# saltoricristiano/lidog

Hardware: AMD Instinct MI355X
Metric: LiDAR scans/sec, MinkUNet34+BEV training step @120k pts (higher is better)
Workload: dtype f32

## Files before the change

include/lidog_amd.h:

```cpp
#ifndef LIDOG_AMD_H
#define LIDOG_AMD_H

#include <stdint.h>

#ifdef __cplusplus
extern "C" {
#endif

const char *lidog_last_error(void);
int lidog_abi_version(void);


int64_t lidog_hash_capacity(int64_t n);

int lidog_coords_insert(const int32_t *coords, int64_t n, uint64_t *keys, int32_t *vals, int64_t cap,
                        int32_t *first_row, int64_t *n_unique_dev, int32_t *err_flag, void *stream);
int lidog_coords_insert_info(const int32_t *coords, int64_t n, uint64_t *keys, int32_t *vals, int64_t cap,
                             int32_t *first_row, int64_t *info, int32_t *err_flag, void *stream);

int lidog_coords_compact(const int32_t *first_row, int64_t n, const uint64_t *keys, int32_t *vals, int64_t cap,
                         const int32_t *coords, int32_t *unique_rows, int32_t *inverse, int32_t *scan_ws,
                         void *stream);

int lidog_coords_stride(const int32_t *coords_in, int64_t n_in, int32_t new_stride, uint64_t *keys,
                        int32_t *vals, int64_t cap, int32_t *parent2child, int32_t *coords_out,
                        int64_t *n_out_dev, int32_t *ws, int32_t *err_flag, void *stream);

int64_t lidog_bitmap_words(int32_t nx, int32_t ny, int32_t nz, int32_t nb, int64_t max_bytes);
int lidog_bitmap_set(const int32_t *coords, int64_t n, int32_t x0, int32_t y0, int32_t z0, int32_t nx, int32_t ny,
                     int32_t nz, int32_t stride, int32_t nb, uint32_t *bits, int32_t *err_flag, void *stream);
int lidog_kernel_map_bits(const int32_t *coords_out, int64_t n_out, const uint64_t *in_keys, const int32_t *in_vals,
                          int64_t in_cap, const int32_t *offsets_host, int32_t K, const uint32_t *bits, int32_t x0,
                          int32_t y0, int32_t z0, int32_t nx, int32_t ny, int32_t nz, int32_t stride, int32_t nb,
                          int32_t *nbr, void *stream);
int lidog_kernel_map_subset(const int32_t *nbr_big, int64_t n, int32_t K_big, const int32_t *sel_host, int32_t K,
                            int32_t *nbr, void *stream);

int lidog_kernel_map(const int32_t *coords_out, int64_t n_out, const uint64_t *in_keys, const int32_t *in_vals,
                     int64_t in_cap, const int32_t *offsets_host, int32_t K, int32_t *nbr, void *stream);

int lidog_kernel_map_pairs(const int32_t *nbr, int64_t n_out, int64_t n_in, int32_t K, int64_t *k_off_dev,
                           int32_t *pair_in, int32_t *pair_out, int32_t *pos_out, int32_t *pos_in, int32_t *ws,
                           void *stream);
int lidog_kernel_map_rows(const int32_t *pos, int64_t n, int32_t K, int32_t mark_k, int32_t *row_ptr,
                          int32_t *row_list, int32_t *ws, void *stream);


int lidog_sconv_gemm(const float *A, const int32_t *gather, const float *B, const float *bias,
                     const int32_t *tile_k, const int32_t *tile_row0, const int32_t *tile_rows, int32_t n_tiles,
                     int32_t Cin, int32_t Cout, float *T, const int32_t *scatter, int64_t a_rows, void *stream);
int32_t lidog_sconv_gemm_units(int32_t multi, int32_t slots);
int lidog_sconv_gemm_addend(const float *A, const int32_t *gather, const float *B, const int32_t *tile_k,
                            const int32_t *tile_row0, const int32_t *tile_rows, int32_t n_tiles, int32_t Cin,
                            int32_t Cout, const float *addend, float *T, const int32_t *scatter, void *stream);

int lidog_sconv_reduce(const float *T, const int32_t *pos, int64_t n, int32_t K, int32_t C, const float *bias,
                       const float *addend ,
                       float *out, void *stream);

int64_t lidog_sconv_reduce_stats_ws(int64_t n, int32_t C);
int lidog_sconv_reduce_stats(const float *T, const int32_t *pos, int64_t n, int32_t K, int32_t C, const float *bias,
                             float *out, double *sums, double *partial_ws, double count, float eps, float momentum,
                             float *mean, float *invstd, float *running_mean, float *running_var, void *stream);
int lidog_sconv_reduce_rows(const float *T, const int32_t *row_ptr, const int32_t *row_list, int64_t n, int32_t C,
                            const float *bias, const float *addend, float *out, void *stream);
int lidog_sconv_reduce_rows_stats(const float *T, const int32_t *row_ptr, const int32_t *row_list, int64_t n,
                                  int32_t C, const float *bias, float *out, double *sums, double *partial_ws,
                                  double count, float eps, float momentum, float *mean, float *invstd,
                                  float *running_mean, float *running_var, void *stream);
int lidog_sconv_reduce_rows_bwdstats(const float *T, const int32_t *row_ptr, const int32_t *row_list, int64_t n,
                                     int32_t C, const float *addend, float *out, const float *pre,
                                     const float *relu_y, const uint32_t *relu_bits, const float *mean,
                                     const float *invstd, const float *relu_w, const float *relu_b, double *sums,
                                     double *partial_ws, double count, float *dw, float *db, void *stream);
int lidog_sconv_reduce_rows_bn(const float *T, const int32_t *row_ptr, const int32_t *row_list, int64_t n, int32_t C,
                               const float *bias, const float *mean, const float *invstd, const float *w,
                               const float *b, const float *residual, int32_t relu, float *out, void *stream);

int lidog_sconv_cin1(const float *x, const int32_t *nbr, const float *W, const float *bias, int64_t n, int32_t K,
                     int32_t C, float *out, void *stream);

int lidog_sconv_wgrad(const float *A, const int32_t *pair_a, const float *G, const int32_t *pair_g,
                      const int32_t *items, int32_t n_items, const int32_t *item_off, int32_t K, int32_t Cin,
                      int32_t Cout, float *partial, float *gW, void *stream);

int lidog_sconv_wgrad_slabs(int32_t Cin, int32_t Cout, int32_t n_items);
int32_t lidog_sconv_wgrad_slots(int32_t Cin, int32_t Cout, int32_t fold);

int lidog_set_sparse_core(int32_t core);
int lidog_get_sparse_core(void);

int lidog_transpose_kernel(const float *W, int32_t K, int32_t Cin, int32_t Cout, float *Wt, void *stream);
int lidog_transpose_batched(const float *src, float *dst, const int64_t *desc, int32_t n_mats, int64_t total_tiles,
                            void *stream);


int64_t lidog_bn_reduce_ws(int32_t C, int64_t hw);
int lidog_bn_stats(const float *x, int64_t n, int32_t C, int64_t hw, double *sums, double *ws, double count,
                   float eps, float momentum, float *mean, float *invstd, float *running_mean, float *running_var,
                   void *stream);
int lidog_bn_finalize(const double *sums, double count, int32_t C, float eps, float momentum, float *mean,
                      float *invstd, float *running_mean, float *running_var, void *stream);
int lidog_bn_apply(const float *x, int64_t n, int32_t C, int64_t hw, const float *mean, const float *invstd,
                   const float *w, const float *b, const float *residual, int32_t relu, float *y, void *stream);
int32_t lidog_stats_max_blocks(void);
int64_t lidog_bn_bwd_reduce_blocks(int64_t n, int32_t C);
int lidog_bn_bwd_reduce(const float *dy, const float *x, const float *relu_y, int64_t n, int32_t C, int64_t hw,
                        const float *mean, const float *invstd, double *sums, double *ws, double count, float *dw,
                        float *db, const float *relu_w, const float *relu_b, void *stream);
int lidog_bn_bwd_apply(const float *dy, const float *x, const float *relu_y, int64_t n, int32_t C, int64_t hw,
                       const float *mean, const float *invstd, const float *w, const double *sums, double count,
                       float *dx, float *dres, float *dw, float *db, const float *relu_b, void *stream);
int64_t lidog_relu_bits_words(int64_t n, int32_t C);
int lidog_bn_apply_bits(const float *x, int64_t n, int32_t C, int64_t hw, const float *mean, const float *invstd,
                        const float *w, const float *b, const float *residual, int32_t relu, float *y,
                        uint32_t *relu_bits, void *stream);
int lidog_bn_apply_sync(const float *x, int64_t n, int32_t C, const double *sums, float eps, float momentum, float *mean,
                        float *invstd, float *running_mean, float *running_var, const float *w, const float *b,
                        const float *residual, int32_t relu, float *y, uint32_t *relu_bits, void *stream);
int lidog_bn_bwd_reduce_bits(const float *dy, const float *x, const float *relu_y, const uint32_t *relu_bits, int64_t n,
                             int32_t C, int64_t hw, const float *mean, const float *invstd, double *sums, double *ws,
                             double count, float *dw, float *db, const float *relu_w, const float *relu_b,
                             void *stream);
int lidog_bn_bwd_apply_bits(const float *dy, const float *x, const float *relu_y, const uint32_t *relu_bits, int64_t n,
                            int32_t C, int64_t hw, const float *mean, const float *invstd, const float *w,
                            const double *sums, double count, float *dx, float *dres, float *dw, float *db,
                            const float *relu_b, void *stream);
int lidog_colsum(const float *x, int64_t n, int32_t C, float *out, double *ws, void *stream);
int64_t lidog_colsum_ws(int32_t C);
int lidog_bn_eval_invstd(const float *running_var, float eps, int32_t C, float *invstd, void *stream);
int lidog_cat2(const float *a, int32_t Ca, const float *b, int32_t Cb, int64_t n, float *out, void *stream);
int lidog_split2(const float *g, int32_t Ca, int32_t Cb, int64_t n, float *ga, float *gb, void *stream);
int lidog_relu_fwd(const float *x, int64_t n, float *y, void *stream);
int lidog_relu_bwd(const float *dy, const float *y, int64_t n, float *dx, void *stream);
int lidog_add(const float *a, const float *b, int64_t n, float *out, void *stream);

int lidog_bev_winner(const int32_t *coords, int64_t n, const int32_t *lut_x, const int32_t *lut_y, int32_t lut_lo,
                     int32_t lut_n, int32_t H, int32_t W, int32_t *winner ,
                     int32_t *pixel , void *stream);
int lidog_bev_pool_fwd(const float *feats, int32_t C, const int32_t *winner, const int32_t *pixel, int64_t n,
                       int32_t B, int32_t H, int32_t W, int32_t pk, int32_t ps, int32_t pp, int32_t Ho, int32_t Wo,
                       float *out ,
                       int32_t *argsrc , uint64_t *rowbits,
                       void *stream);
int lidog_bev_pool_bwd(const float *gout , const int32_t *argsrc, const int32_t *winner,
                       const int32_t *pixel, int64_t n, int32_t C, int32_t B, int32_t H, int32_t W, int32_t pk,
                       int32_t ps, int32_t pp, int32_t Ho, int32_t Wo, float *gfeats , void *stream);

int lidog_conv2d_fwd(const float *x, const float *w, const float *bias, int32_t B, int32_t Cin, int32_t H,
                     int32_t W, int32_t Cout, int32_t ksize, int32_t stride, int32_t pad, float *y, void *stream);
int lidog_conv2d_dgrad(const float *gy, const float *w, int32_t B, int32_t Cin, int32_t H, int32_t W,
                       int32_t Cout, int32_t ksize, int32_t stride, int32_t pad, float *gx, float *ws,
                       void *stream);
int lidog_conv2d_wgrad(const float *x, const float *gy, int32_t B, int32_t Cin, int32_t H, int32_t W,
                       int32_t Cout, int32_t ksize, int32_t stride, int32_t pad, float *gw, float *gbias,
                       float *ws, int64_t ws_floats, void *stream);

int64_t lidog_conv2d_support_ws(int32_t B, int32_t Cin, int32_t H, int32_t W);
int lidog_conv2d_support(const int32_t *support, int32_t B, int32_t Cin, int32_t H, int32_t W, int32_t *act,
                         void *stream);
int lidog_conv2d_fwd_sparse(const float *x, const float *w, const int32_t *act, int32_t B, int32_t Cin, int32_t H,
                            int32_t W, int32_t Cout, float *y, float *ws, void *stream);
int lidog_conv2d_dgrad_sparse(const float *gy, const float *w, const int32_t *act, int32_t B, int32_t Cin, int32_t H,
                              int32_t W, int32_t Cout, float *gx, float *ws, void *stream);
int lidog_conv2d_support_work(const int32_t *act, int32_t B, int32_t Cin, int32_t H, int32_t W, int32_t Cout,
                              double *out, void *stream);
int64_t lidog_conv2d_wgrad_sparse_ws(int32_t B, int32_t Cin, int32_t H, int32_t W, int32_t Cout);
int lidog_conv2d_wgrad_sparse(const float *x, const float *gy, const int32_t *act, int32_t B, int32_t Cin, int32_t H,
                              int32_t W, int32_t Cout, float *gw, float *ws, int64_t ws_floats, void *stream);

int64_t lidog_dice_ws(int32_t C);
int lidog_dice_fwd(const float *logits, const int64_t *target, int64_t n, int32_t C, int64_t ignore_label,
                   int32_t has_ignore, float eps, int32_t soft, int32_t powerize, int32_t use_tmask, float offset,
                   double *ws, float *loss, float *coef, void *stream);
int lidog_dice_bwd(const float *logits, const int64_t *target, int64_t n, int32_t C, int64_t ignore_label,
                   int32_t has_ignore, float eps, int32_t soft, int32_t powerize, const float *coef, const float *gout,
                   float *glogits, void *stream);
int lidog_dice_kitti_fwd(const float *logits, const int64_t *target, int64_t n, int32_t C, int64_t ignore_label,
                         int32_t has_ignore, float eps, int32_t powerize, int32_t use_tmask, float offset, double *ws,
                         float *loss, float *coef, void *stream);
int lidog_dice_kitti_bwd(const float *logits, const int64_t *target, int64_t n, int32_t C, int64_t ignore_label,
                         int32_t has_ignore, float eps, int32_t powerize, const float *coef, const float *gout,
                         float *glogits, void *stream);

int64_t lidog_ce_ws(int32_t C);
int lidog_ce_fwd(const float *logits, const int64_t *target, int64_t n, int32_t C, int64_t ignore_label,
                 int32_t has_ignore, const float *weight, int32_t focal, double alpha, double gamma, double *ws,
                 float *loss, float *coef, void *stream);
int lidog_ce_bwd(const float *logits, const int64_t *target, int64_t n, int32_t C, int64_t ignore_label,
                 int32_t has_ignore, const float *weight, const float *coef, const float *gout, float *glogits,
                 void *stream);

int lidog_voxel_floor(const float *points, int64_t n, float qx, float qy, float qz, int32_t batch, int32_t *rows,
                      void *stream);
int lidog_label_vote(const int32_t *labels, const int32_t *unique_rows, const int32_t *inverse, int64_t n, int64_t m,
                     int32_t ignore_label, int32_t *voxel_labels, void *stream);
int lidog_bev_label_raster(const int32_t *coords, const int32_t *labels, int64_t n, const int32_t *lut_x,
                           const int32_t *lut_y, const int32_t *lut_z, int32_t lut_lo, int32_t lut_n, int32_t B,
                           int32_t S, const int64_t *batch_start, int32_t *point_idx, int64_t *img_labels,
                           void *stream);

int lidog_adam_step(float *param, const float *grad, float *exp_avg, float *exp_avg_sq, int64_t n, float lr,
                    float beta1, float beta2, float eps, float weight_decay, int32_t step, float grad_scale,
                    void *stream);
int lidog_grad_accumulate(const int64_t *segs, int32_t n_segs, void *stream);
int lidog_sgd_step(float *param, const float *grad, float *momentum_buf, int64_t n, float lr, float momentum,
                   float weight_decay, int32_t nesterov, float grad_scale, void *stream);

int32_t lidog_comm_unique_id_bytes(void);
int lidog_comm_unique_id(void *id_out);
int lidog_comm_init_rank(const void *id, int32_t nranks, int32_t rank, void **comm_out);
int lidog_comm_destroy(void *comm);
int32_t lidog_comm_count(void *comm);
int lidog_allreduce_f32(float *buf, int64_t n, void *comm, void *stream);
int lidog_allreduce_f64(double *buf, int64_t n, void *comm, void *stream);

int32_t lidog_peer_handle_bytes(void);
int64_t lidog_peer_mailbox_bytes(int32_t nranks, int32_t max_doubles);
int lidog_peer_mailbox_alloc(int64_t bytes, void **ptr_out, void *handle_out);
int lidog_peer_mailbox_open(const void *handle, void **ptr_out);
int lidog_peer_comm_create(int32_t rank, int32_t nranks, int32_t max_doubles, void *local, void *const *peer_ptrs,
                           void **comm_out);
int32_t lidog_peer_max_doubles(void *comm);
int lidog_peer_set_spin_limit(void *comm, int64_t polls );
int lidog_peer_allreduce_f64(void *comm, double *buf, int64_t n, void *stream);
int32_t lidog_peer_status(void *comm);
int lidog_peer_comm_destroy(void *comm, int32_t close_peers);
int lidog_peer_rebind_stream(void *comm, void *stream);
int64_t lidog_peer_calls(void *comm);
int lidog_peer_inject_skip_flag(void *comm, int64_t seq);
int lidog_peer_mailbox_free(void *ptr);
int lidog_peer_mailbox_close(void *peer_ptr);

int64_t lidog_kernel_map_sorted_ws(int64_t n);
int lidog_kernel_map_sorted(const int32_t *nbr, int64_t n, int32_t K, const int64_t *k_off, int32_t *perm,
                            uint32_t *wave_masks, int32_t *tile_order, void *ws, int64_t ws_bytes, void *stream);
int lidog_sconv_os(const float *A, const int32_t *nbr, int64_t n, int32_t K, const int32_t *perm,
                   const uint32_t *wave_masks, const int32_t *tile_order, const float *W, int32_t reverse,
                   const float *bias, const float *addend, int32_t Cin, int32_t Cout, float *out, void *stream);
int64_t lidog_sconv_os_stats_ws(int64_t n, int32_t C);
// ... 178 lines not shown
```

lidog_amd/_lib.py:

```python
import ctypes
import os

import torch

_HERE = os.path.dirname(os.path.abspath(__file__))
SO_PATH = os.environ.get("LIDOG_SO") or os.path.join(_HERE, "_C", "liblidog_amd.so")

_i32, _i64, _p, _f, _d = ctypes.c_int32, ctypes.c_int64, ctypes.c_void_p, ctypes.c_float, ctypes.c_double

SIGNATURES = {
    "lidog_abi_version": [],
    "lidog_hash_capacity": [_i64],
    "lidog_coords_insert": [_p, _i64, _p, _p, _i64, _p, _p, _p, _p],
    "lidog_coords_insert_info": [_p, _i64, _p, _p, _i64, _p, _p, _p, _p],
    "lidog_coords_compact": [_p, _i64, _p, _p, _i64, _p, _p, _p, _p, _p],
    "lidog_coords_stride": [_p, _i64, _i32, _p, _p, _i64, _p, _p, _p, _p, _p, _p],
    "lidog_kernel_map": [_p, _i64, _p, _p, _i64, _p, _i32, _p, _p],
    "lidog_bitmap_words": [_i32, _i32, _i32, _i32, _i64],
    "lidog_bitmap_set": [_p, _i64, _i32, _i32, _i32, _i32, _i32, _i32, _i32, _i32, _p, _p, _p],
    "lidog_kernel_map_bits": [_p, _i64, _p, _p, _i64, _p, _i32, _p, _i32, _i32, _i32, _i32, _i32, _i32, _i32, _i32, _p, _p],
    "lidog_kernel_map_pairs": [_p, _i64, _i64, _i32, _p, _p, _p, _p, _p, _p, _p],
    "lidog_sconv_gemm_units": [_i32, _i32],
    "lidog_sconv_gemm": [_p, _p, _p, _p, _p, _p, _p, _i32, _i32, _i32, _p, _p, _i64, _p],
    "lidog_sconv_gemm_addend": [_p, _p, _p, _p, _p, _p, _i32, _i32, _i32, _p, _p, _p, _p],
    "lidog_sconv_reduce": [_p, _p, _i64, _i32, _i32, _p, _p, _p, _p],
    "lidog_sconv_reduce_stats_ws": [_i64, _i32],
    "lidog_sconv_reduce_stats": [_p, _p, _i64, _i32, _i32, _p, _p, _p, _p, _d, _f, _f, _p, _p, _p, _p, _p],
    "lidog_kernel_map_rows": [_p, _i64, _i32, _i32, _p, _p, _p, _p],
    "lidog_sconv_reduce_rows": [_p, _p, _p, _i64, _i32, _p, _p, _p, _p],
    "lidog_sconv_reduce_rows_bn": [_p, _p, _p, _i64, _i32, _p, _p, _p, _p, _p, _p, _i32, _p, _p],
    "lidog_sconv_reduce_rows_stats": [_p, _p, _p, _i64, _i32, _p, _p, _p, _p, _d, _f, _f, _p, _p, _p, _p, _p],
    "lidog_sconv_reduce_rows_bwdstats": [_p, _p, _p, _i64, _i32, _p, _p, _p, _p, _p, _p, _p, _p, _p, _p, _p, _d, _p, _p, _p],
    "lidog_bn_bwd_reduce_blocks": [_i64, _i32],
    "lidog_stats_max_blocks": [],
    "lidog_sconv_cin1": [_p, _p, _p, _p, _i64, _i32, _i32, _p, _p],
    "lidog_kernel_map_subset": [_p, _i64, _i32, _p, _i32, _p, _p],
    "lidog_kernel_map_sorted_ws": [_i64],
    "lidog_kernel_map_sorted": [_p, _i64, _i32, _p, _p, _p, _p, _p, _i64, _p],
    "lidog_sconv_os": [_p, _p, _i64, _i32, _p, _p, _p, _p, _i32, _p, _p, _i32, _i32, _p, _p],
    "lidog_sconv_os_stats_ws": [_i64, _i32],
    "lidog_sconv_os_bn": [_p, _p, _i64, _i32, _p, _p, _p, _p, _p, _i32, _i32, _p, _p, _p, _p, _p, _i32, _p, _p],
    "lidog_sconv_os_stats": [_p, _p, _i64, _i32, _p, _p, _p, _p, _p, _i32, _i32, _p, _p, _p, _d, _f, _f, _p, _p, _p, _p, _p],
    "lidog_pack_kernels_bf16": [_p, _p, _p, _i32, _i64, _p],
    "lidog_sconv_gemm_bf16": [_p, _p, _p, _p, _p, _p, _p, _i32, _i32, _i32, _p, _p, _p],
    "lidog_sconv_os_bn_bf16": [_p, _p, _i64, _i32, _p, _p, _p, _p, _p, _i32, _i32, _p, _p, _p, _p, _p, _i32, _p, _p],
    "lidog_sconv_wgrad_bf16": [_p, _p, _p, _p, _p, _i32, _p, _i32, _i32, _i32, _p, _p, _p],
    "lidog_sconv_wgrad_bf16_slabs": [_i32, _i32, _i32],
    "lidog_sconv_wgrad_bf16_slots": [_i32, _i32],
    "lidog_sconv_wgrad": [_p, _p, _p, _p, _p, _i32, _p, _i32, _i32, _i32, _p, _p, _p],
    "lidog_sconv_gemm_in_bn": [_p, _p, _p, _p, _p, _p, _p, _i32, _i32, _i32, _p, _p, _p, _p, _p, _p, _i32, _i64, _p],
    "lidog_sconv_os_stats_in_bn": [_p, _p, _i64, _i32, _p, _p, _p, _p, _p, _i32, _i32, _p, _p, _p, _d, _f, _f, _p, _p, _p, _p,
                                   _p, _p, _p, _p, _i32, _p],
    "lidog_sconv_wgrad_in_bn": [_p, _p, _p, _p, _p, _i32, _p, _i32, _i32, _i32, _p, _p, _p, _p, _p, _p, _i32, _p],
    "lidog_sconv_wgrad_slabs": [_i32, _i32, _i32],
    "lidog_sconv_wgrad_slots": [_i32, _i32, _i32],
    "lidog_set_sparse_core": [_i32],
    "lidog_get_sparse_core": [],
    "lidog_transpose_kernel": [_p, _i32, _i32, _i32, _p, _p],
    "lidog_transpose_batched": [_p, _p, _p, _i32, _i64, _p],
    "lidog_bn_reduce_ws": [_i32, _i64],
    "lidog_bn_stats": [_p, _i64, _i32, _i64, _p, _p, _d, _f, _f, _p, _p, _p, _p, _p],
    "lidog_bn_finalize": [_p, _d, _i32, _f, _f, _p, _p, _p, _p, _p],
    "lidog_bn_apply": [_p, _i64, _i32, _i64, _p, _p, _p, _p, _p, _i32, _p, _p],
    "lidog_bn_bwd_reduce": [_p, _p, _p, _i64, _i32, _i64, _p, _p, _p, _p, _d, _p, _p, _p, _p, _p],
    "lidog_bn_bwd_apply": [_p, _p, _p, _i64, _i32, _i64, _p, _p, _p, _p, _d, _p, _p, _p, _p, _p, _p],
    "lidog_relu_bits_words": [_i64, _i32],
    "lidog_bn_apply_bits": [_p, _i64, _i32, _i64, _p, _p, _p, _p, _p, _i32, _p, _p, _p],
    "lidog_bn_bwd_reduce_bits": [_p, _p, _p, _p, _i64, _i32, _i64, _p, _p, _p, _p, _d, _p, _p, _p, _p, _p],
    "lidog_bn_bwd_apply_bits": [_p, _p, _p, _p, _i64, _i32, _i64, _p, _p, _p, _p, _d, _p, _p, _p, _p, _p, _p],
    "lidog_colsum": [_p, _i64, _i32, _p, _p, _p],
    "lidog_colsum_ws": [_i32],
    "lidog_bn_eval_invstd": [_p, _f, _i32, _p, _p],
    "lidog_cat2": [_p, _i32, _p, _i32, _i64, _p, _p],
    "lidog_split2": [_p, _i32, _i32, _i64, _p, _p, _p],
    "lidog_relu_fwd": [_p, _i64, _p, _p],
    "lidog_relu_bwd": [_p, _p, _i64, _p, _p],
    "lidog_add": [_p, _p, _i64, _p, _p],
    "lidog_bev_winner": [_p, _i64, _p, _p, _i32, _i32, _i32, _i32, _p, _p, _p],
    "lidog_bev_pool_fwd": [_p, _i32, _p, _p, _i64, _i32, _i32, _i32, _i32, _i32, _i32, _i32, _i32, _p, _p, _p, _p],
    "lidog_bev_pool_bwd": [_p, _p, _p, _p, _i64, _i32, _i32, _i32, _i32, _i32, _i32, _i32, _i32, _i32, _p, _p],
    "lidog_conv2d_fwd": [_p, _p, _p, _i32, _i32, _i32, _i32, _i32, _i32, _i32, _i32, _p, _p],
    "lidog_conv2d_dgrad": [_p, _p, _i32, _i32, _i32, _i32, _i32, _i32, _i32, _i32, _p, _p, _p],
    "lidog_conv2d_wgrad": [_p, _p, _i32, _i32, _i32, _i32, _i32, _i32, _i32, _i32, _p, _p, _p, _i64, _p],
    "lidog_conv2d_support_ws": [_i32, _i32, _i32, _i32],
    "lidog_conv2d_support": [_p, _i32, _i32, _i32, _i32, _p, _p],
    "lidog_conv2d_fwd_sparse": [_p, _p, _p, _i32, _i32, _i32, _i32, _i32, _p, _p, _p],
    "lidog_conv2d_dgrad_sparse": [_p, _p, _p, _i32, _i32, _i32, _i32, _i32, _p, _p, _p],
    "lidog_conv2d_wgrad_sparse_ws": [_i32, _i32, _i32, _i32, _i32],
    "lidog_conv2d_wgrad_sparse": [_p, _p, _p, _i32, _i32, _i32, _i32, _i32, _p, _p, _i64, _p],
    "lidog_voxel_floor": [_p, _i64, _f, _f, _f, _i32, _p, _p],
    "lidog_label_vote": [_p, _p, _p, _i64, _i64, _i32, _p, _p],
    "lidog_bev_label_raster": [_p, _p, _i64, _p, _p, _p, _i32, _i32, _i32, _i32, _p, _p, _p, _p],
    "lidog_dice_ws": [_i32],
    "lidog_dice_fwd": [_p, _p, _i64, _i32, _i64, _i32, _f, _i32, _i32, _i32, _f, _p, _p, _p, _p],
    "lidog_dice_bwd": [_p, _p, _i64, _i32, _i64, _i32, _f, _i32, _i32, _p, _p, _p, _p],
    "lidog_dice_kitti_fwd": [_p, _p, _i64, _i32, _i64, _i32, _f, _i32, _i32, _f, _p, _p, _p, _p],
    "lidog_dice_kitti_bwd": [_p, _p, _i64, _i32, _i64, _i32, _f, _i32, _p, _p, _p, _p],
    "lidog_ce_ws": [_i32],
    "lidog_ce_fwd": [_p, _p, _i64, _i32, _i64, _i32, _p, _i32, _d, _d, _p, _p, _p, _p],
    "lidog_ce_bwd": [_p, _p, _i64, _i32, _i64, _i32, _p, _p, _p, _p, _p],
    "lidog_adam_step": [_p, _p, _p, _p, _i64, _f, _f, _f, _f, _f, _i32, _f, _p],
    "lidog_sgd_step": [_p, _p, _p, _i64, _f, _f, _f, _i32, _f, _p],
    "lidog_comm_unique_id_bytes": [],
    "lidog_comm_unique_id": [_p],
    "lidog_comm_init_rank": [_p, _i32, _i32, ctypes.POINTER(ctypes.c_void_p)],
    "lidog_comm_destroy": [_p],
    "lidog_allreduce_f32": [_p, _i64, _p, _p],
    "lidog_allreduce_f64": [_p, _i64, _p, _p],
    "lidog_comm_count": [_p],
    "lidog_peer_handle_bytes": [],
    "lidog_peer_mailbox_bytes": [_i32, _i32],
    "lidog_peer_mailbox_alloc": [_i64, ctypes.POINTER(ctypes.c_void_p), _p],
    "lidog_peer_mailbox_open": [_p, ctypes.POINTER(ctypes.c_void_p)],
    "lidog_peer_comm_create": [_i32, _i32, _i32, _p, _p, ctypes.POINTER(ctypes.c_void_p)],
    "lidog_peer_max_doubles": [_p],
    "lidog_peer_set_spin_limit": [_p, _i64],
    "lidog_peer_allreduce_f64": [_p, _p, _i64, _p],
    "lidog_peer_status": [_p],
    "lidog_peer_comm_destroy": [_p, _i32],
    "lidog_peer_rebind_stream": [_p, _p],
    "lidog_peer_calls": [_p],
    "lidog_peer_inject_skip_flag": [_p, _i64],
    "lidog_peer_mailbox_free": [_p],
    "lidog_peer_mailbox_close": [_p],
    "lidog_tiles_host": [_p, _i32, _i32, _i32, _p, _i64],
    "lidog_wgrad_items_host": [_p, _i32, _i64, _i32, _i32, _p, _p, _i64],
    "lidog_conv2d_support_work": [_p, _i32, _i32, _i32, _i32, _i32, _p, _p],
    "lidog_bn_apply_sync": [_p, _i64, _i32, _p, _f, _f, _p, _p, _p, _p, _p, _p, _p, _i32, _p, _p, _p],
    "lidog_trunk_fusions": [_i32],
    "lidog_trunk_in_bn_readers": [_p, _i32, _p, _i32, _p, _i32, _p, _i32, _p],
    "lidog_trunk_gemm_timing": [_i32],
    "lidog_trunk_gemm_timing_read": [_p],
    "lidog_trunk_work_read": [_p],
    "lidog_trunk_forward": [_p, _p, _i32, _p, _i32, _p, _i32, _p, _i32, _p, _p, _p, _i64, _p, _i64, _p, _p, _i32, _p, _p, _p],
    "lidog_trunk_backward": [_p, _p, _i32, _p, _i32, _p, _i32, _p, _i32, _p, _p, _p, _p, _p, _p, _i64, _p, _i64, _p,
                             _i64, _p, _p, _i32, _i32, _p, _p, _p],
    "lidog_in_segments_ws": [_i64],
    "lidog_in_segments": [_p, _i64, _i32, _p, _p, _p, _p, _i64, _p],
    "lidog_in_reduce_ws": [_i32, _i32],
    "lidog_in_stats": [_p, _i64, _i32, _i32, _p, _p, _f, _p, _p, _p, _p],
    "lidog_in_apply": [_p, _i64, _i32, _i32, _p, _p, _p, _p, _p, _p, _p],
    "lidog_in_bwd_reduce": [_p, _p, _i64, _i32, _i32, _p, _p, _p, _p, _p, _p, _p, _p, _p],
    "lidog_in_bwd_apply": [_p, _p, _i64, _i32, _i32, _p, _p, _p, _p, _p, _p, _p],
    "lidog_ibn_apply": [_p, _i64, _i32, _i32, _p, _p, _p, _p, _p, _p, _p, _p, _p, _p, _p, _p],
    "lidog_ibn_bwd_reduce": [_p, _p, _p, _i64, _i32, _i32, _p, _p, _p, _p, _p, _p, _p, _p, _p, _p, _p, _p, _p, _p, _p],
    "lidog_ibn_bwd_apply": [_p, _p, _p, _i64, _i32, _i32, _p, _p, _p, _p, _d, _p, _p, _p, _p, _p, _p, _p],
    "lidog_iw_ws": [],
    "lidog_iw_fwd": [_p, _p, _p, _p, _i32, _d, _p, _p, _p, _p],
    "lidog_iw_bwd": [_p, _p, _p, _p, _i32, _d, _p, _p, _p],
    "lidog_grad_accumulate": [_p, _i32, _p],
    "lidog_mix_histogram": [_p, _i64, _i32, _p, _p],
    "lidog_mix_split_ws": [_i64, _i32],
    "lidog_mix_split": [_p, _i64, _p, _i32, _i32, _p, _p, _p, _p],
    "lidog_mix_gather": [_p, _i64, _p, _p, _p, _p, _p, _i32, _i64, _f, _p, _i32, _p, _p, _p],
    "lidog_mix_gather_aug": [_p, _i64, _p, _i64, _p, _p, _p, _p, _i32, _i64, _f, _p, _i32, _p, _i32, _d, _d, _d, _p, _i32,
                             _p, _p, _p],
    "lidog_dbscan_ws": [_i64],
    "lidog_dbscan": [_p, _i64, _f, _d, _i32, _p, _p, _p, _i64, _p],
    "lidog_cluster_boxes": [_p, _p, _i64, _i32, _p, _p, _p, _p],
    "lidog_sn_scale_coords": [_p, _i64, _f, _f, _f, _f, _p, _p],
    "lidog_augment_is_f64": [_p, _i32],
    "lidog_augment_ws": [_i64],
    "lidog_augment_points": [_p, _i64, _p, _i64, _p, _p, _i32, _i32, _d, _d, _d, _i32, _p, _p, _p, _p, _p, _p, _p, _p],
    "lidog_eval_confusion": [_p, _p, _p, _i64, _i32, _i32, _i64, _p, _p, _p, _p],
    "lidog_eval_pack_ws": [_i64, _i32],
    "lidog_eval_pack": [_p, _p, _p, _i64, _i32, _i64, _p, _p, _p, _p],
    "lidog_train_confusion": [_p, _p, _p, _i32, _i32, _i64, _p, _p, _p],
    "lidog_scan_load_ws": [_i64],
    "lidog_scan_load": [_p, _i32, _p, _i32, _i32, _i64, _p, _i32, _i32, _f, _p, _p, _p, _i32, _p, _p, _p],
    "lidog_scan_keep_rows_ws": [_i64],
    "lidog_scan_keep_rows": [_p, _i32, _i64, _i32, _f, _p, _p, _p, _p],
    "lidog_point_labels_ws": [_i64],
    "lidog_point_labels": [_p, _i64, _i32, _i32, _p, _p, _p, _i64, _i64, _p, _p, _p, ctypes.c_uint32, _p, _i32, _i32, _p,
                           _i32, _i64, _p, _p, _p, _p, _p],
    "lidog_pool_rows": [_p, _p, _p, _p, _i64, _i32, _i32, _p, _p, _p],
    "lidog_pool_rows_max": [_p, _p, _p, _p, _i64, _i32, _p, _p, _p],
    "lidog_pool_rows_max_bwd": [_p, _p, _p, _p, _p, _i64, _i32, _p, _p],
    "lidog_pool_global_ws": [_i64, _i32, _i32],
    "lidog_pool_global": [_p, _i64, _i32, _i32, _p, _p, _i32, _p, _p, _p, _i64, _p],
    "lidog_pool_global_bwd": [_p, _p, _i64, _i32, _i32, _p, _p, _i32, _p, _p],
}
_RESTYPES = {"lidog_hash_capacity": _i64, "lidog_sconv_reduce_stats_ws": _i64, "lidog_bn_reduce_ws": _i64,
             "lidog_dice_ws": _i64, "lidog_ce_ws": _i64, "lidog_colsum_ws": _i64, "lidog_conv2d_support_ws": _i64, "lidog_conv2d_wgrad_sparse_ws": _i64,
             "lidog_tiles_host": _i64, "lidog_wgrad_items_host": _i64, "lidog_bitmap_words": _i64,
             "lidog_bn_bwd_reduce_blocks": _i64, "lidog_relu_bits_words": _i64,
             "lidog_peer_mailbox_bytes": _i64, "lidog_peer_calls": _i64,
             "lidog_kernel_map_sorted_ws": _i64, "lidog_sconv_os_stats_ws": _i64, "lidog_in_segments_ws": _i64,
             "lidog_in_reduce_ws": _i64, "lidog_iw_ws": _i64, "lidog_mix_split_ws": _i64,
             "lidog_dbscan_ws": _i64, "lidog_augment_ws": _i64, "lidog_eval_pack_ws": _i64,
             "lidog_scan_load_ws": _i64, "lidog_pool_global_ws": _i64, "lidog_scan_keep_rows_ws": _i64,
             "lidog_point_labels_ws": _i64}

ABI_VERSION = 8

_lib = None


def load():
    global _lib
    if _lib is None:
        if not os.path.exists(SO_PATH):
            raise RuntimeError(
                f"{SO_PATH} is missing: build it with `python -m lidog_amd.build` (hipcc, gfx950). "
                "lidog_amd has no CPU or torch fallback.")
        L = ctypes.CDLL(SO_PATH)
        L.lidog_last_error.restype = ctypes.c_char_p
        L.lidog_last_error.argtypes = []
        have = L.lidog_abi_version()
# ... 52 lines not shown
```

lidog_amd/csrc/sconv_mfma.hip:

```cpp
#include <stdlib.h>

#include "common.h"
#include "sconv_mfma.h"
#include "clock_stamp.h"

typedef float f32x16 __attribute__((ext_vector_type(16)));

#define MG_TM 128
#define MG_BK 32
#define MG_SA 33

template <int NT>
__device__ __forceinline__ void frag_load(const float *p, float (&f)[NT]) {
    if constexpr (NT == 4) {
        float4 v = *reinterpret_cast<const float4 *>(p);
        f[0] = v.x; f[1] = v.y; f[2] = v.z; f[3] = v.w;
    } else if constexpr (NT == 2) {
        float2 v = *reinterpret_cast<const float2 *>(p);
        f[0] = v.x; f[1] = v.y;
    } else {
#pragma unroll
        for (int t = 0; t < NT; ++t) f[t] = p[t];
    }
}
// ... 461 lines not shown
    constexpr int TPW = (TILES + WPG - 1) / WPG;
    __shared__ __attribute__((aligned(16))) float As[MW_R * TM];
    __shared__ __attribute__((aligned(16))) float Gs[MW_R * TN];
    const int item = items[3 * n_items + blockIdx.x];
    const int tiles_n = Cout / TN;
    const int ci0 = (blockIdx.y / tiles_n) * TM, co0 = (blockIdx.y % tiles_n) * TN;
    const int tid = threadIdx.x, lane = tid & 63, wave = tid >> 6;
    const int li = lane & 31, kh = lane >> 5;
    LIDOG_STAMP_BEGIN()
    const int grp = wave / WPG, wig = wave % WPG;
    const int64_t p0 = items[n_items + item], p1 = items[2 * n_items + item];

    int a_off[TPW], g_off[TPW];
    bool own[TPW];
#pragma unroll
    for (int t = 0; t < TPW; ++t) {
        int tt = wig * TPW + t;
        own[t] = tt < TILES;
        int mi = own[t] ? tt % MT : 0, nj = own[t] ? tt / MT : 0;
        a_off[t] = 32 * mi + li;
        g_off[t] = 32 * nj + li;
    }
    f32x16 acc[TPW];
#pragma unroll
    for (int t = 0; t < TPW; ++t)
#pragma unroll
        for (int e = 0; e < 16; ++e) acc[t][e] = 0.f;

    constexpr int AV = (MW_R * TM / 4 + NTH - 1) / NTH, GV = (MW_R * TN / 4 + NTH - 1) / NTH;
    float4 ra[AV], rg[GV];
    int ia[AV], ig[GV];
    auto load_idx = [&](int64_t p) {
#pragma unroll
        for (int j = 0; j < AV; ++j) {
            int f = tid + NTH * j;
            f = f < MW_R * TM / 4 ? f : MW_R * TM / 4 - 1;
            int64_t pr = p + f / (TM / 4);
            ia[j] = pa[pr < p1 ? pr : p1 - 1];
        }
#pragma unroll
        for (int j = 0; j < GV; ++j) {
            int f = tid + NTH * j;
            f = f < MW_R * TN / 4 ? f : MW_R * TN / 4 - 1;
            int64_t pr = p + f / (TN / 4);
            ig[j] = pg[pr < p1 ? pr : p1 - 1];
        }
    };
    auto load_rows = [&](int64_t p) {
#pragma unroll
        for (int j = 0; j < AV; ++j) {
            int f = tid + NTH * j;
            f = f < MW_R * TM / 4 ? f : MW_R * TM / 4 - 1;
            int r = f / (TM / 4), c4 = f % (TM / 4);
            (void)r;
            ra[j] = *reinterpret_cast<const float4 *>(A + (size_t)ia[j] * Cin + ci0 + c4 * 4);
        }
#pragma unroll
        for (int j = 0; j < GV; ++j) {
            int f = tid + NTH * j;
            f = f < MW_R * TN / 4 ? f : MW_R * TN / 4 - 1;
            int r = f / (TN / 4), c4 = f % (TN / 4);
            (void)r;
            rg[j] = *reinterpret_cast<const float4 *>(G + (size_t)ig[j] * Cout + co0 + c4 * 4);
        }
    };
    if (p0 < p1) {
        load_idx(p0);
        load_rows(p0);
        load_idx(p0 + MW_R);
    }
    if constexpr (FOLD) {
        for (int i = tid; i < TM; i += NTH) {
            s_par[i] = in_bn.mean[ci0 + i];
            s_par[TM + i] = in_bn.invstd[ci0 + i];
            s_par[2 * TM + i] = in_bn.w[ci0 + i];
            s_par[3 * TM + i] = in_bn.b[ci0 + i];
        }
    }
    for (int64_t p = p0; p < p1; p += MW_R) {
        __syncthreads();
#pragma unroll
        for (int j = 0; j < AV; ++j) {
            int f = tid + NTH * j;
            const bool ok = p + f / (TM / 4) < p1;
            float4 v = ra[j];
            if constexpr (FOLD) {
                const int c = ((f < MW_R * TM / 4 ? f : MW_R * TM / 4 - 1) % (TM / 4)) * 4;
                v = in_bn_apply(v, *reinterpret_cast<const float4 *>(&s_par[c]),
                                *reinterpret_cast<const float4 *>(&s_par[TM + c]),
                                *reinterpret_cast<const float4 *>(&s_par[2 * TM + c]),
                                *reinterpret_cast<const float4 *>(&s_par[3 * TM + c]), in_bn.relu);
            }
            if (f < MW_R * TM / 4) *reinterpret_cast<float4 *>(&As[f * 4]) = make_float4(ok ? v.x : 0.f, ok ? v.y : 0.f, ok ? v.z : 0.f, ok ? v.w : 0.f);
        }
#pragma unroll
        for (int j = 0; j < GV; ++j) {
            int f = tid + NTH * j;
            const bool ok = p + f / (TN / 4) < p1;
            if (f < MW_R * TN / 4) *reinterpret_cast<float4 *>(&Gs[f * 4]) = make_float4(ok ? rg[j].x : 0.f, ok ? rg[j].y : 0.f, ok ? rg[j].z : 0.f, ok ? rg[j].w : 0.f);
        }
        __syncthreads();
        if (p + MW_R < p1) {
            load_rows(p + MW_R);
            load_idx(p + 2 * MW_R);
        }
        constexpr int Q = MW_R / 2 / NGRP;
        float af[TPW], gf[TPW], an[TPW], gn[TPW];
        {
            const int kk = 2 * grp + kh;
#pragma unroll
            for (int t = 0; t < TPW; ++t) {
                af[t] = As[kk * TM + a_off[t]];
                gf[t] = Gs[kk * TN + g_off[t]];
            }
        }
#pragma unroll
        for (int q = 0; q < Q; ++q) {
            if (q + 1 < Q) {
                const int kk = 2 * ((q + 1) * NGRP + grp) + kh;
#pragma unroll
                for (int t = 0; t < TPW; ++t) {
                    an[t] = As[kk * TM + a_off[t]];
                    gn[t] = Gs[kk * TN + g_off[t]];
                }
            }
            __builtin_amdgcn_sched_barrier(0);
#pragma unroll
            for (int t = 0; t < TPW; ++t) acc[t] = __builtin_amdgcn_mfma_f32_32x32x2f32(af[t], gf[t], acc[t], 0, 0, 0);
            __builtin_amdgcn_sched_barrier(0);
            if (q + 1 < Q) {
#pragma unroll
                for (int t = 0; t < TPW; ++t) {
                    af[t] = an[t];
                    gf[t] = gn[t];
                }
            }
        }
    }
    float *dst = partial + (size_t)(item * NGRP + grp) * Cin * Cout;
#pragma unroll
    for (int t = 0; t < TPW; ++t) {
        if (!own[t]) continue;
        int tt = wig * TPW + t;
        int mi = tt % MT, nj = tt / MT;
#pragma unroll
        for (int e = 0; e < 16; ++e) {
            int ci = ci0 + 32 * mi + (e & 3) + 8 * (e >> 2) + 4 * kh;
            dst[(size_t)ci * Cout + co0 + 32 * nj + li] = acc[t][e];
        }
    }
    LIDOG_STAMP_END()
}

static int tile32(int C) { return (C % 128 == 0) ? 4 : (C % 96 == 0) ? 3 : (C % 64 == 0) ? 2 : 1; }

static void wg_shape(int tiles, int *nw, int *ngrp) {
    switch (tiles) {
        case 1: *nw = 4; *ngrp = 4; break;
        case 2: *nw = 4; *ngrp = 2; break;
        case 3: case 6: case 9: *nw = 3; *ngrp = 1; break;
        default: *nw = 4; *ngrp = 1;
    }
}

int lidog_wgrad_mfma_slabs(int Cin, int Cout, int n_items) {
    int nw, ngrp;
    wg_shape(tile32(Cin) * tile32(Cout), &nw, &ngrp);
    return n_items * ngrp;
}

template <int MT, int NT, int NW, int NGRP>
static void launch_wg(dim3 grid, hipStream_t st, const float *A, const int32_t *pa, const float *G, const int32_t *pg,
                      const int32_t *items, int n_items, int Cin, int Cout, float *partial, InBn in_bn) {
    if (in_bn.mean)
        k_sconv_wgrad_mfma<MT, NT, NW, NGRP, true><<<grid, 64 * NW, 0, st>>>(A, pa, G, pg, items, n_items, Cin, Cout,
                                                                             partial, in_bn);
    else
        k_sconv_wgrad_mfma<MT, NT, NW, NGRP, false><<<grid, 64 * NW, 0, st>>>(A, pa, G, pg, items, n_items, Cin, Cout,
                                                                              partial, in_bn);
}

template <int MT, int NT, int NW, int NGRP>
static int occ_wg(bool fold) {
    int n = 0;
    hipError_t e = fold ? hipOccupancyMaxActiveBlocksPerMultiprocessor(&n, k_sconv_wgrad_mfma<MT, NT, NW, NGRP, true>, 64 * NW, 0)
                        : hipOccupancyMaxActiveBlocksPerMultiprocessor(&n, k_sconv_wgrad_mfma<MT, NT, NW, NGRP, false>, 64 * NW, 0);
    return e == hipSuccess ? n : -1;
}

int lidog_wgrad_mfma_wg_per_cu(int Cin, int Cout, int fold) {
    int mt = tile32(Cin), nt = tile32(Cout);
#define WG(MT_, NT_, NW_, NG_) return occ_wg<MT_, NT_, NW_, NG_>(fold != 0)
    switch (mt * 10 + nt) {
        case 11: WG(1, 1, 4, 4);
        case 12: WG(1, 2, 4, 2);
        case 21: WG(2, 1, 4, 2);
        case 13: WG(1, 3, 3, 1);
        case 31: WG(3, 1, 3, 1);
        case 14: WG(1, 4, 4, 1);
        case 41: WG(4, 1, 4, 1);
        case 22: WG(2, 2, 4, 1);
        case 23: WG(2, 3, 3, 1);
        case 32: WG(3, 2, 3, 1);
        case 24: WG(2, 4, 4, 1);
        case 42: WG(4, 2, 4, 1);
        case 33: WG(3, 3, 3, 1);
        case 34: WG(3, 4, 4, 1);
        case 43: WG(4, 3, 4, 1);
        default: WG(4, 4, 4, 1);
    }
#undef WG
}

int lidog_launch_wgrad_mfma(const float *A, const int32_t *pa, const float *G, const int32_t *pg,
                            const int32_t *items, int n_items, int Cin, int Cout, float *partial, InBn in_bn,
                            hipStream_t st) {
    int mt = tile32(Cin), nt = tile32(Cout);
    dim3 grid((unsigned)n_items, (unsigned)((Cin / (32 * mt)) * (Cout / (32 * nt))));
#define WG(MT_, NT_, NW_, NG_) launch_wg<MT_, NT_, NW_, NG_>(grid, st, A, pa, G, pg, items, n_items, Cin, Cout, partial, in_bn)
    switch (mt * 10 + nt) {
        case 11: WG(1, 1, 4, 4); break;
        case 12: WG(1, 2, 4, 2); break;
        case 21: WG(2, 1, 4, 2); break;
        case 13: WG(1, 3, 3, 1); break;
        case 31: WG(3, 1, 3, 1); break;
        case 14: WG(1, 4, 4, 1); break;
        case 41: WG(4, 1, 4, 1); break;
        case 22: WG(2, 2, 4, 1); break;
        case 23: WG(2, 3, 3, 1); break;
        case 32: WG(3, 2, 3, 1); break;
        case 24: WG(2, 4, 4, 1); break;
        case 42: WG(4, 2, 4, 1); break;
        case 33: WG(3, 3, 3, 1); break;
        case 34: WG(3, 4, 4, 1); break;
        case 43: WG(4, 3, 4, 1); break;
        default: WG(4, 4, 4, 1);
    }
#undef WG
    return 0;
}
```

Before: 86.71.

## Add LDS ring-buffered wgrad MFMA kernel with async global-to-LDS DMA for 32x32

Adds a new weight-gradient kernel that stages gathered A and G rows into a multi-stage LDS ring using global_load_lds direct DMA, with pair indices prefetched ahead and row loads interleaved between MFMA issues. Out-of-range rows read from a device zero row. By default it is selected only for non-folded Cin=Cout=32 layers, and a runtime override picks 2 or 3 stages. The aim is to hide gather latency behind MFMA work, at the cost of more LDS use, hand-written waitcnt bookkeeping and possibly lower occupancy.

After: 86.73, median of 4. No clear change (+0.0%).

```diff
diff --git a/include/lidog_amd.h b/include/lidog_amd.h
--- a/include/lidog_amd.h
+++ b/include/lidog_amd.h
@@ -86,6 +86,9 @@
 
 int lidog_sconv_wgrad_slabs(int32_t Cin, int32_t Cout, int32_t n_items);
 int32_t lidog_sconv_wgrad_slots(int32_t Cin, int32_t Cout, int32_t fold);
+
+int32_t lidog_sconv_wgrad_ring(int32_t form);
+int32_t lidog_zero_row_nonzeros(void);
 
 int lidog_set_sparse_core(int32_t core);
 int lidog_get_sparse_core(void);
diff --git a/lidog_amd/_lib.py b/lidog_amd/_lib.py
--- a/lidog_amd/_lib.py
+++ b/lidog_amd/_lib.py
@@ -54,6 +54,8 @@
     "lidog_sconv_wgrad_in_bn": [_p, _p, _p, _p, _p, _i32, _p, _i32, _i32, _i32, _p, _p, _p, _p, _p, _p, _i32, _p],
     "lidog_sconv_wgrad_slabs": [_i32, _i32, _i32],
     "lidog_sconv_wgrad_slots": [_i32, _i32, _i32],
+    "lidog_sconv_wgrad_ring": [_i32],
+    "lidog_zero_row_nonzeros": [],
     "lidog_set_sparse_core": [_i32],
     "lidog_get_sparse_core": [],
     "lidog_transpose_kernel": [_p, _i32, _i32, _i32, _p, _p],
diff --git a/lidog_amd/csrc/sconv_mfma.hip b/lidog_amd/csrc/sconv_mfma.hip
--- a/lidog_amd/csrc/sconv_mfma.hip
+++ b/lidog_amd/csrc/sconv_mfma.hip
@@ -637,6 +637,224 @@
     LIDOG_STAMP_END()
 }
 
+
+__device__ __attribute__((aligned(16))) float g_zero_row[128];
+
+extern "C" int32_t lidog_zero_row_nonzeros(void) {
+    uint32_t host[128];
+    if (hipMemcpyFromSymbol(host, HIP_SYMBOL(g_zero_row), sizeof(host)) != hipSuccess) return -1;
+    int32_t n = 0;
+    for (int i = 0; i < 128; ++i) n += host[i] != 0u;
+    return n;
+}
+
+__device__ __forceinline__ unsigned ring_lds_addr(const void *p) {
+    return __builtin_amdgcn_readfirstlane((unsigned)(size_t)(__attribute__((address_space(3))) const char *)p);
+}
+__device__ __forceinline__ void ring_dma16(const void *gsrc, unsigned lds_dst) {
+    unsigned keep;
+    asm volatile("s_mov_b32 %0, m0\n\ts_mov_b32 m0, %2\n\ts_nop 0\n\tglobal_load_lds_dwordx4 %1, off\n\ts_mov_b32 m0, %0"
+                 : "=&s"(keep) : "v"(gsrc), "s"(lds_dst) : "memory");
+}
+__device__ __forceinline__ void ring_dma4(const void *gsrc, unsigned lds_dst) {
+    unsigned keep;
+    asm volatile("s_mov_b32 %0, m0\n\ts_mov_b32 m0, %2\n\ts_nop 0\n\tglobal_load_lds_dword %1, off\n\ts_mov_b32 m0, %0"
+                 : "=&s"(keep) : "v"(gsrc), "s"(lds_dst) : "memory");
+}
+#define RING_MAX_WAIT 24
+__device__ __forceinline__ void ring_wait_vm(int n) {
+#define RW(N_) case N_: asm volatile("s_waitcnt vmcnt(" #N_ ")" ::: "memory"); break;
+    switch (n) {
+        RW(1) RW(2) RW(3) RW(4) RW(5) RW(6) RW(7) RW(8) RW(9) RW(10) RW(11) RW(12)
+        RW(13) RW(14) RW(15) RW(16) RW(17) RW(18) RW(19) RW(20) RW(21) RW(22) RW(23) RW(24)
+        default: asm volatile("s_waitcnt vmcnt(0)" ::: "memory");
+    }
+#undef RW
+}
+__device__ __forceinline__ void ring_barrier() { asm volatile("s_waitcnt lgkmcnt(0)\n\ts_barrier" ::: "memory"); }
+
+template <int MT, int NT, int NW, int NGRP, bool FOLD, int R, int S>
+__global__ __launch_bounds__(64 * NW) void k_sconv_wgrad_ring(const float *__restrict__ A, const int32_t *__restrict__ pa,
+                                                              const float *__restrict__ G, const int32_t *__restrict__ pg,
+                                                              const int32_t *__restrict__ items, int n_items, int Cin,
+                                                              int Cout, float *__restrict__ partial, InBn in_bn) {
+    constexpr int TM = 32 * MT, TN = 32 * NT, NTH = 64 * NW;
+    constexpr int TILES = MT * NT;
+    constexpr int WPG = NW / NGRP, TPW = (TILES + WPG - 1) / WPG;
+    constexpr int PA = R * TM / 256, PG = R * TN / 256;
+    constexpr int AV = (PA + NW - 1) / NW, GV = (PG + NW - 1) / NW;
+    constexpr int LA = S - 1;
+    constexpr int NI = 8;
+    static_assert(R % (2 * NGRP) == 0 && R <= 32 && LA >= 1 && LA <= 3 && LA + 2 <= NI, "ring shape");
+    static_assert((LA - 1) * (AV + GV + 1) <= RING_MAX_WAIT, "ring_wait_vm range");
+    __shared__ __attribute__((aligned(1024))) float As[S * R * TM];
+    __shared__ __attribute__((aligned(1024))) float Gs[S * R * TN];
+    __shared__ __attribute__((aligned(256))) int32_t Is[NI * 64];
+    __shared__ __attribute__((aligned(16))) float s_par[FOLD ? 4 * TM : 4];
+    const int item = items[3 * n_items + blockIdx.x];
+    const int tiles_n = Cout / TN;
+    const int ci0 = (blockIdx.y / tiles_n) * TM, co0 = (blockIdx.y % tiles_n) * TN;
+    const int tid = threadIdx.x, lane = tid & 63, wave = __builtin_amdgcn_readfirstlane(tid >> 6);
+    const int li = lane & 31, kh = lane >> 5;
+    LIDOG_STAMP_BEGIN()
+    const int grp = wave / WPG, wig = wave % WPG;
+    const int64_t p0 = items[n_items + item], p1 = items[2 * n_items + item];
+    const int nc = p0 < p1 ? (int)((p1 - p0 + R - 1) / R) : 0;
+
+    int a_off[TPW], g_off[TPW];
+    bool own[TPW];
+#pragma unroll
+    for (int t = 0; t < TPW; ++t) {
+        int tt = wig * TPW + t;
+        own[t] = tt < TILES;
+        int mi = own[t] ? tt % MT : 0, nj = own[t] ? tt / MT : 0;
+        a_off[t] = 32 * mi + li;
+        g_off[t] = 32 * nj + li;
+    }
+    f32x16 acc[TPW];
+#pragma unroll
+    for (int t = 0; t < TPW; ++t)
+#pragma unroll
+        for (int e = 0; e < 16; ++e) acc[t][e] = 0.f;
+
+    const int n_w = (wave < PA ? (PA - wave + NW - 1) / NW : 0) + (wave < PG ? (PG - wave + NW - 1) / NW : 0);
+    auto dma_idx = [&](int c) {
+        int64_t pr = p0 + (int64_t)c * R + (li < R ? li : R - 1);
+        pr = pr < p1 ? pr : p1 - 1;
+        ring_dma4((kh ? pg : pa) + pr, ring_lds_addr(&Is[(c % NI) * 64]));
+    };
+    const float *const zero_row = g_zero_row;
+    int ia[AV], ig[GV];
+    auto read_idx = [&](int c) {
+        const int32_t *is = &Is[(c % NI) * 64];
+#pragma unroll
+        for (int j = 0; j < AV; ++j) ia[j] = is[((wave + NW * j < PA ? wave + NW * j : 0) * 64 + lane) / (TM / 4)];
+#pragma unroll
+        for (int j = 0; j < GV; ++j) ig[j] = is[32 + ((wave + NW * j < PG ? wave + NW * j : 0) * 64 + lane) / (TN / 4)];
+    };
+    auto piece = [&](int c, int j) {
+        const int64_t pc = p0 + (int64_t)c * R;
+        if (j < AV) {
+            const int u = wave + NW * j;
+            if (u < PA) {
+                const int f = u * 64 + lane, r = f / (TM / 4), c4 = f % (TM / 4);
+                const float *src = A + (size_t)ia[j] * Cin + ci0;
+                ring_dma16((pc + r < p1 ? src : zero_row) + c4 * 4, ring_lds_addr(&As[(c % S) * R * TM + u * 256]));
+            }
+        } else {
+            const int u = wave + NW * (j - AV);
+            if (u < PG) {
+                const int f = u * 64 + lane, r = f / (TN / 4), c4 = f % (TN / 4);
+                const float *src = G + (size_t)ig[j - AV] * Cout + co0;
+                ring_dma16((pc + r < p1 ? src : zero_row) + c4 * 4, ring_lds_addr(&Gs[(c % S) * R * TN + u * 256]));
+            }
+        }
+    };
+    auto dma_rows = [&](int c) {
+        read_idx(c);
+#pragma unroll
+        for (int j = 0; j < AV + GV; ++j) piece(c, j);
+    };
+    if constexpr (FOLD) {
+        for (int i = tid; i < TM; i += NTH) {
+            s_par[i] = in_bn.mean[ci0 + i];
+            s_par[TM + i] = in_bn.invstd[ci0 + i];
+            s_par[2 * TM + i] = in_bn.w[ci0 + i];
+            s_par[3 * TM + i] = in_bn.b[ci0 + i];
+        }
+    }
+    if (nc > 0) {
+        if (wave == 0)
+            for (int c = 0; c <= LA + 1; ++c) dma_idx(c);
+        asm volatile("s_waitcnt vmcnt(0)" ::: "memory");
+        ring_barrier();
+        for (int c = 0; c < LA && c < nc; ++c) dma_rows(c);
+    }
+    for (int t = 0; t < nc; ++t) {
+        const int k = nc - 1 - t < LA - 1 ? nc - 1 - t : LA - 1;
+        int allow = k * n_w;
+        if (wave == 0)
+            for (int c = t + 2; c <= t + k; ++c) allow += c >= LA;
+        ring_wait_vm(allow);
+        float *as = &As[(t % S) * R * TM], *gs = &Gs[(t % S) * R * TN];
+        if constexpr (FOLD) {
+            const int64_t pc = p0 + (int64_t)t * R;
+#pragma unroll
+            for (int j = 0; j < AV; ++j) {
+                const int u = wave + NW * j;
+                if (u < PA) {
+                    const int f = u * 64 + lane, r = f / (TM / 4), c = (f % (TM / 4)) * 4;
+                    const bool ok = pc + r < p1;
+                    float4 v = *reinterpret_cast<const float4 *>(&as[f * 4]);
+                    v = in_bn_apply(v, *reinterpret_cast<const float4 *>(&s_par[c]),
+                                    *reinterpret_cast<const float4 *>(&s_par[TM + c]),
+                                    *reinterpret_cast<const float4 *>(&s_par[2 * TM + c]),
+                                    *reinterpret_cast<const float4 *>(&s_par[3 * TM + c]), in_bn.relu);
+                    *reinterpret_cast<float4 *>(&as[f * 4]) = make_float4(ok ? v.x : 0.f, ok ? v.y : 0.f, ok ? v.z : 0.f, ok ? v.w : 0.f);
+                }
+            }
+        }
+        ring_barrier();
+        const bool more = t + LA < nc;
+        if (more) {
+            if (wave == 0) dma_idx(t + LA + 2);
+            read_idx(t + LA);
+        }
+        constexpr int Q = R / 2 / NGRP;
+        float af[TPW], gf[TPW], an[TPW], gn[TPW];
+        {
+            const int kk = 2 * grp + kh;
+#pragma unroll
+            for (int t2 = 0; t2 < TPW; ++t2) {
+                af[t2] = as[kk * TM + a_off[t2]];
+                gf[t2] = gs[kk * TN + g_off[t2]];
+            }
+        }
+#pragma unroll
+        for (int q = 0; q < Q; ++q) {
+            if (q + 1 < Q) {
+                const int kk = 2 * ((q + 1) * NGRP + grp) + kh;
+#pragma unroll
+                for (int t2 = 0; t2 < TPW; ++t2) {
+                    an[t2] = as[kk * TM + a_off[t2]];
+                    gn[t2] = gs[kk * TN + g_off[t2]];
+                }
+            }
+            __builtin_amdgcn_sched_barrier(0);
+#pragma unroll
+            for (int t2 = 0; t2 < TPW; ++t2) acc[t2] = __builtin_amdgcn_mfma_f32_32x32x2f32(af[t2], gf[t2], acc[t2], 0, 0, 0);
+            __builtin_amdgcn_sched_barrier(0);
+            if (more) {
+                if (q < AV + GV) piece(t + LA, q);
+                if constexpr (AV + GV > Q)
+                    if (q == Q - 1)
+#pragma unroll
+                        for (int j = Q; j < AV + GV; ++j) piece(t + LA, j);
+            }
+            if (q + 1 < Q) {
+#pragma unroll
+                for (int t2 = 0; t2 < TPW; ++t2) {
+                    af[t2] = an[t2];
+                    gf[t2] = gn[t2];
+                }
+            }
+        }
+    }
+    float *dst = partial + (size_t)(item * NGRP + grp) * Cin * Cout;
+#pragma unroll
+    for (int t = 0; t < TPW; ++t) {
+        if (!own[t]) continue;
+        int tt = wig * TPW + t;
+        int mi = tt % MT, nj = tt / MT;
+#pragma unroll
+        for (int e = 0; e < 16; ++e) {
+            int ci = ci0 + 32 * mi + (e & 3) + 8 * (e >> 2) + 4 * kh;
+            dst[(size_t)ci * Cout + co0 + 32 * nj + li] = acc[t][e];
+        }
+    }
+    LIDOG_STAMP_END()
+}
+
 static int tile32(int C) { return (C % 128 == 0) ? 4 : (C % 96 == 0) ? 3 : (C % 64 == 0) ? 2 : 1; }
 
 static void wg_shape(int tiles, int *nw, int *ngrp) {
@@ -654,28 +872,56 @@
     return n_items * ngrp;
 }
 
+static int g_wgrad_ring = -1;
+
+extern "C" int32_t lidog_sconv_wgrad_ring(int32_t form) {
+    const int32_t old = g_wgrad_ring;
+    g_wgrad_ring = form < 0 ? -1 : (form > 2 ? 2 : form);
+    return old;
+}
+
+static int ring_form(int Cin, int Cout, bool fold) {
+    if (g_wgrad_ring >= 0) return g_wgrad_ring;
+    if (fold) return 0;
+    if (Cin == 32 && Cout == 32) return 1;
+    return 0;
+}
+
+typedef void (*wg_fn)(const float *, const int32_t *, const float *, const int32_t *, const int32_t *, int, int, int, float *,
+                      InBn);
+
+template <int MT, int NT, int NW, int NGRP, bool FOLD>
+static wg_fn wg_kernel_f(int form) {
+    switch (form) {
+        case 1: return k_sconv_wgrad_ring<MT, NT, NW, NGRP, FOLD, 32, 3>;
+        case 2: return k_sconv_wgrad_ring<MT, NT, NW, NGRP, FOLD, 32, 2>;
+        default: return k_sconv_wgrad_mfma<MT, NT, NW, NGRP, FOLD>;
+    }
+}
+
+template <int MT, int NT, int NW, int NGRP>
+static wg_fn wg_kernel(int Cin, int Cout, bool fold) {
+    const int form = ring_form(Cin, Cout, fold);
+    return fold ? wg_kernel_f<MT, NT, NW, NGRP, true>(form) : wg_kernel_f<MT, NT, NW, NGRP, false>(form);
+}
+
 template <int MT, int NT, int NW, int NGRP>
 static void launch_wg(dim3 grid, hipStream_t st, const float *A, const int32_t *pa, const float *G, const int32_t *pg,
                       const int32_t *items, int n_items, int Cin, int Cout, float *partial, InBn in_bn) {
-    if (in_bn.mean)
-        k_sconv_wgrad_mfma<MT, NT, NW, NGRP, true><<<grid, 64 * NW, 0, st>>>(A, pa, G, pg, items, n_items, Cin, Cout,
-                                                                             partial, in_bn);
-    else
-        k_sconv_wgrad_mfma<MT, NT, NW, NGRP, false><<<grid, 64 * NW, 0, st>>>(A, pa, G, pg, items, n_items, Cin, Cout,
-                                                                              partial, in_bn);
+    wg_kernel<MT, NT, NW, NGRP>(Cin, Cout, in_bn.mean != nullptr)<<<grid, 64 * NW, 0, st>>>(A, pa, G, pg, items, n_items, Cin, Cout,
+                                                                                 partial, in_bn);
 }
 
 template <int MT, int NT, int NW, int NGRP>
-static int occ_wg(bool fold) {
+static int occ_wg(int Cin, int Cout, bool fold) {
     int n = 0;
-    hipError_t e = fold ? hipOccupancyMaxActiveBlocksPerMultiprocessor(&n, k_sconv_wgrad_mfma<MT, NT, NW, NGRP, true>, 64 * NW, 0)
-                        : hipOccupancyMaxActiveBlocksPerMultiprocessor(&n, k_sconv_wgrad_mfma<MT, NT, NW, NGRP, false>, 64 * NW, 0);
+    hipError_t e = hipOccupancyMaxActiveBlocksPerMultiprocessor(&n, wg_kernel<MT, NT, NW, NGRP>(Cin, Cout, fold), 64 * NW, 0);
     return e == hipSuccess ? n : -1;
 }
 
 int lidog_wgrad_mfma_wg_per_cu(int Cin, int Cout, int fold) {
     int mt = tile32(Cin), nt = tile32(Cout);
-#define WG(MT_, NT_, NW_, NG_) return occ_wg<MT_, NT_, NW_, NG_>(fold != 0)
+#define WG(MT_, NT_, NW_, NG_) return occ_wg<MT_, NT_, NW_, NG_>(Cin, Cout, fold != 0)
     switch (mt * 10 + nt) {
         case 11: WG(1, 1, 4, 4);
         case 12: WG(1, 2, 4, 2);
```
